# princeton-computational-imaging/Neural-Volume-Super-Resolution

Hardware: AMD Instinct MI355X
Metric: rendered rays/sec (64+128 samples) at 800x800 Lego-like view (higher is better)
Workload: dtype f32 as 2 f16 limbs (3 MFMA products, f32 acc); 1 GPU; Blender-'lego'-like 800x800 view, 64 coarse + 128 fine samples, tri-plane decoder (3x800^2x48 + 32^2x48 planes, 4+4x128 MLP), 1 view per GPU per step; partition=view

## Files before the change

neural-volume-super-resolution_amd/csrc/pair_core.h:

```cpp
#pragma once
#include <type_traits>
#include <utility>

#ifndef R3_DMA_AUX
#define R3_DMA_AUX 0
#endif
#ifndef R3_ABLATE
#define R3_ABLATE 0
#endif
#include "limb_core.h"
#include "side_work.h"

#ifndef R3_GATHER_NT
#define R3_GATHER_NT 0
#endif
#ifndef R3_STAMP
#define R3_STAMP 0
#endif
#if R3_STAMP == 4
#define R3_MARK(i)
#define R3_MARKB(i)
#define R3_RESET
#define R3_MARKH(i) { __builtin_amdgcn_sched_barrier(0); const unsigned long long t_ = __builtin_amdgcn_s_memtime(); stamp[i] += (float)(t_ - tprev); tprev = t_; __builtin_amdgcn_sched_barrier(0); }
#define R3_RESETH { tprev = __builtin_amdgcn_s_memtime(); }
#elif R3_STAMP == 3
#define R3_MARKH(i)
#define R3_RESETH
#define R3_MARK(i)
#define R3_MARKB(i) { __builtin_amdgcn_sched_barrier(0); const unsigned long long t_ = __builtin_amdgcn_s_memtime(); stamp[i] += (float)(t_ - tprev); tprev = t_; __builtin_amdgcn_sched_barrier(0); }
#define R3_RESET { tprev = __builtin_amdgcn_s_memtime(); }
#elif R3_STAMP
#define R3_MARKB(i)
#define R3_RESET
#define R3_MARKH(i)
#define R3_RESETH
#define R3_MARK(i) { __builtin_amdgcn_sched_barrier(0); const unsigned long long t_ = __builtin_amdgcn_s_memtime(); stamp[i] += (float)(t_ - tprev); tprev = t_; __builtin_amdgcn_sched_barrier(0); }
#else
#define R3_MARK(i)
#define R3_MARKB(i)
#define R3_RESET
#define R3_MARKH(i)
#define R3_RESETH
#endif
#ifndef R3_RELU_PK
#define R3_RELU_PK 0
#endif
#ifndef R3_BLEND_PK
#define R3_BLEND_PK 0
#endif
#ifndef R3_NO_VIEW_HOIST
#define R3_NO_VIEW_HOIST 1
#endif

namespace nvsr {

template <int LIMBS>
struct Lds3 {
    static constexpr bool F16 = limb_f16(LIMBS);
    static constexpr int SLOT = 4 * kb_words(LIMBS);
    static constexpr int SMALL = 2 * SLOT;
    static constexpr int RAYS = SMALL + SMALL_FLOATS;
    static constexpr int RAY_FLOATS = F16 ? 8 : 20;
    static constexpr int TAP_FLOATS = F16 ? 8 : 0;
    static constexpr int VTAPS = RAYS + RAYS2 * RAY_FLOATS;
    static constexpr int FAR = F16 ? VTAPS + RAYS2 * TAP_FLOATS : -1;
    static constexpr int RES = VTAPS + RAYS2 * TAP_FLOATS + (F16 ? RAYS2 : 0);
    static constexpr int RES_KB = F16 ? 9 : 0;
    static constexpr int PTS_WORDS = 8 * RAYS2;
    static constexpr int PTS = F16 ? VTAPS : RES + RES_KB * kb_words(LIMBS);
    static_assert(!F16 || RAYS2 * TAP_FLOATS >= PTS_WORDS, "the points' region fits the taps'");
    static constexpr int TOTAL = RES + RES_KB * kb_words(LIMBS) + (F16 ? 0 : PTS_WORDS);
};
static_assert(Lds3<3>::TOTAL * 4 <= 160 * 1024 && Lds3<2>::TOTAL * 4 <= 160 * 1024 && Lds3<1>::TOTAL * 4 <= 160 * 1024, "LDS budget");

struct Tile3 {
    f32x16 acc[4];
    f32x16 act[4];
    float D[HALF_C], F[HALF_C];
    float V[HALF_C];
    float T, cr, cg, cb, dep, ac, zc, zn;
    float raw[4];
};

struct RawTaps4 { f32x4 r[4][HALF_C / 4]; };
constexpr int GATHER_STEPS = 12 + HALF_C;
__device__ __forceinline__ void gather4_load(int k, const GatherJob& job, int h, RawTaps4& rt) {
    const int tap = k / 3, i0 = 2 * (k % 3);
#if R3_ABLATE & 1
    rt.r[tap][i0] = f32x4{job.t.nw, job.t.ne, job.t.sw, job.t.se};
    rt.r[tap][i0 + 1] = f32x4{job.t.se, job.t.ne, job.t.sw, job.t.nw};
    return;
#endif
    const int off = tap == 0 ? job.t.o00 : tap == 1 ? job.t.o01 : tap == 2 ? job.t.o10 : job.t.o11;
    const f32x4* p = reinterpret_cast<const f32x4*>(job.plane + off + HALF_C * h);
    rt.r[tap][i0] = p[i0];
    rt.r[tap][i0 + 1] = p[i0 + 1];
}
__device__ __forceinline__ void gather4_blend(int c, const GatherJob& job, const RawTaps4& rt, float (&F)[HALF_C]) {
    const int i = c >> 2, j = c & 3;
    F[c] = fmaf(rt.r[3][i][j], job.t.se, fmaf(rt.r[2][i][j], job.t.sw, fmaf(rt.r[1][i][j], job.t.ne, rt.r[0][i][j] * job.t.nw)));
}

template <int NS, bool LOADS, bool BLENDS, bool PK = false>
__device__ __forceinline__ void gather_roll(int slot, const GatherJob& jl, float (&Fl)[HALF_C], const GatherJob& jb, float (&Fb)[HALF_C], int h,
                                            RawTaps4& rt) {
    spread<72, 0, NS>(slot, [&](int v) {
        if (LOADS && v % 3 == 0) {
            const int tap = (v / 3) / 6, piece = (v / 3) % 6;
#if R3_ABLATE & 1
            rt.r[tap][piece] = f32x4{jl.t.nw, jl.t.ne, jl.t.sw, jl.t.se};
#else
            int off = tap == 0 ? jl.t.o00 : tap == 1 ? jl.t.o01 : tap == 2 ? jl.t.o10 : jl.t.o11;
#if R3_ABLATE & 2
            off = __builtin_amdgcn_readfirstlane(off);
#endif
#if R3_ABLATE & 4
            off = off & 0xffff;
            off -= off % 48;
#endif
#if R3_GATHER_NT
            rt.r[tap][piece] = __builtin_nontemporal_load(reinterpret_cast<const f32x4*>(jl.plane + off + HALF_C * h) + piece);
#else
            rt.r[tap][piece] = reinterpret_cast<const f32x4*>(jl.plane + off + HALF_C * h)[piece];
#endif
#endif
        }
        const int w = v / 18, u = v % 18;
        if constexpr (PK) {
            if (u % 3 != 2) {
                const int c = 2 * ((u / 3) * 2 + u % 3);
                if (LOADS && w == 3) {
                    f32x2_t m = f32x2_t{rt.r[0][c >> 2][c & 3], rt.r[0][c >> 2][(c & 3) + 1]} * f32x2_t{jl.t.nw, jl.t.nw};
                    Fl[c] = m[0]; Fl[c + 1] = m[1];
                }
                if (BLENDS && w < 3) {
                    const float wt = w == 0 ? jb.t.ne : w == 1 ? jb.t.sw : jb.t.se;
                    f32x2_t f = f32x2_t{Fb[c], Fb[c + 1]};
                    f32x2_t m = __builtin_elementwise_fma(f32x2_t{rt.r[w + 1][c >> 2][c & 3], rt.r[w + 1][c >> 2][(c & 3) + 1]}, f32x2_t{wt, wt}, f);
                    Fb[c] = m[0]; Fb[c + 1] = m[1];
                }
            }
        } else {
#pragma unroll
        for (int c = (u * 4) / 3; c < ((u + 1) * 4) / 3; ++c) {
            if (LOADS && w == 3) Fl[c] = rt.r[0][c >> 2][c & 3] * jl.t.nw;
            if (BLENDS && w < 3) Fb[c] = fmaf(rt.r[w + 1][c >> 2][c & 3], w == 0 ? jb.t.ne : w == 1 ? jb.t.sw : jb.t.se, Fb[c]);
        }
        }
    });
}

template <int NS, bool LOADS, int HL, bool BLENDS, int HB>
__device__ __forceinline__ void gather_half(int slot, const GatherJob& jl, const GatherJob& jb, float (&F)[HALF_C], int h, RawTaps2& rt) {
    if constexpr (BLENDS)
        spread<HALF_C, 0, NS / 2>(slot, [&](int c) {
            const float a = rt.r0[c >> 2][c & 3], b = rt.r1[c >> 2][c & 3];
            if (HB == 0) F[c] = fmaf(b, jb.t.ne, a * jb.t.nw);
            else F[c] = fmaf(b, jb.t.se, fmaf(a, jb.t.sw, F[c]));
        });
    if constexpr (LOADS)
        spread<12, NS / 2, NS>(slot, [&](int k) {
            const int off = HL == 0 ? ((k & 1) ? jl.t.o01 : jl.t.o00) : ((k & 1) ? jl.t.o11 : jl.t.o10);
            const f32x4 v = reinterpret_cast<const f32x4*>(jl.plane + off + HALF_C * h)[k >> 1];
            if (k & 1) rt.r1[k >> 1] = v; else rt.r0[k >> 1] = v;
        });
}

template <int N>
__device__ __forceinline__ void ring3_sync() {
#if R3_ABLATE & 256
#elif R3_ABLATE & 9
    asm volatile("s_waitcnt vmcnt(0)" ::: "memory");
#else
    asm volatile("s_waitcnt vmcnt(%0)" ::"n"(N) : "memory");
#endif
#if !(R3_ABLATE & 64)
    __syncthreads();
#endif
}

constexpr int RELU_STEPS = 68;
#ifndef R3_BOUNCE
#define R3_BOUNCE 0
#endif
typedef __attribute__((address_space(3))) f32x4* lds_f32x4_p;
struct BiasPend4 { f32x4 v[2]; f32x4 a[2]; lds_f32x4_p slot; };
__device__ __forceinline__ lds_f32x4_p bounce_slot(float* p) { return (lds_f32x4_p)p; }
template <int LIMBS>
__device__ __forceinline__ void relu_bias_step(int k, const float* bias, int h, const f32x16 (&acc)[4], f32x16 (&act)[4], BiasPend4& pend, f32x2_t nsc) {
    if ((k & 3) == 0 && k < 64) pend.v[(k >> 2) & 1] = *reinterpret_cast<const f32x4*>(bias + (k >> 2) * 8 + h * 4);
#if R3_BOUNCE
    if constexpr (LIMBS == 2) {
        if ((k & 3) == 0 && k < 64) {
            const int q = k >> 2;
            *pend.slot = f32x4{acc[q >> 2][4 * (q & 3)], acc[q >> 2][4 * (q & 3) + 1], acc[q >> 2][4 * (q & 3) + 2], acc[q >> 2][4 * (q & 3) + 3]};
        }
        if ((k & 3) == 2 && k < 66) {
            asm volatile("" : "+v"(pend.slot));
            pend.a[(k >> 2) & 1] = *pend.slot;
        }
        if (k >= 4) {
            const int r = k - 4;
            float v;
            asm("v_fma_f32 %0, -%1, %2, %3\n\tv_max_i32 %0, 0, %0" : "=v"(v) : "v"(pend.a[(r >> 2) & 1][r & 3]), "s"(nsc[0]), "v"(pend.v[(r >> 2) & 1][r & 3]));
            act[r >> 4][r & 15] = v;
        }
        return;
    }
#endif
#if R3_ABLATE & 2048
    if (k >= 4 && ((k - 4) & 15) != 0) return;
#endif
    if (k >= 4) {
        const int r = k - 4;
        if constexpr (LIMBS == 1) {
            float v, t;
            asm("v_mul_f32 %1, 0, %2\n\tv_fma_f32 %0, -%2, %3, %4\n\tv_add_f32 %0, %0, |%1|\n\tv_max_i32 %0, 0, %0"
                : "=v"(v), "=&v"(t) : "v"(acc[r >> 4][r & 15]), "s"(nsc[0]), "v"(pend.v[(r >> 2) & 1][r & 3]));
            act[r >> 4][r & 15] = v;
        } else if constexpr (LIMBS == 2) {
// ... 84 lines not shown
```

neural-volume-super-resolution_amd/csrc/render3.hip:

```cpp
#include "pair_core.h"

#include "colour_order.h"
#include "occupancy.h"
#include "nvsr_internal.h"

namespace nvsr {

template <int LZ>
__device__ __forceinline__ void render_pass3_body(const SceneDev& sc, const float* __restrict__ packed, long N, int S,
                                                  const float* __restrict__ rays, const float* __restrict__ z, int lindisp,
                                                  const float* __restrict__ noise, int white,
                                                  float* __restrict__ rgb, float* __restrict__ disp,
                                                  float* __restrict__ acc, float* __restrict__ weights,
                                                  float* __restrict__ depth, float* __restrict__ raw_out, unsigned* __restrict__ flag,
                                                  float* __restrict__ live_z = nullptr, float* __restrict__ live_w = nullptr,
                                                  int* __restrict__ live_n = nullptr, const int* __restrict__ group_slot = nullptr,
                                                  const int* __restrict__ pts = nullptr, const int* __restrict__ pt_steps = nullptr, float* views = nullptr,
                                                  const int* __restrict__ kept = nullptr, const int* __restrict__ kept_n = nullptr) {
    constexpr int LIMBS = LZ & 7;
    constexpr bool ZCOMP = (LZ & 8) != 0;
    constexpr int PHASE = (LZ >> 4) & 7;
    constexpr bool FUSED = PHASE == 0, KEPT = PHASE == 4, DENSITY = PHASE == 1 || KEPT, POINTS = PHASE == 3, COLOUR = PHASE == 2 || POINTS;
    constexpr bool F16 = limb_f16(LIMBS);
    using L = Lds3<LIMBS>;
// ... 76 lines not shown
        if constexpr (ZCOMP) return nullptr;
        asm volatile("" : "+v"(ray));
        return z + ray * S;
    };
    int idxX = 0, idxY = 0, idxXn = 0, idxYn = 0, cX = 0, cY = 0;
    bool actX = false, actY = false;
    auto kept_at = [&](const int* kp, int k, int prev) NVSR_INL -> int { const int e = kp[k < S ? k : S - 1]; return e < 0 ? prev : e; };
    auto live_depth = [&](const float* lzp, const float* rc, int n, int k) NVSR_INL -> float {
        if (n == 0) return rc[7];
        const float e = lzp[k < n ? k : n - 1];
        if constexpr (ZCOMP) return depth_of(nullptr, rc, __float_as_int(e));
        else return e;
    };
    auto live_weight = [](const float* lwp, int n, int k) NVSR_INL -> float { return n == 0 ? 0.0f : lwp[k < n ? k : n - 1]; };
    int slotX = ownX, slotY = ownY, slotXn = ownX, slotYn = ownY, eX1 = POINT_NONE, eY1 = POINT_NONE;
    bool liveX = false, liveY = false, liveXn = false, liveYn = false;
    float* const pt_sums = ldsf + L::PTS;
    float* const pt_exch = pt_sums + 3 * RAYS2;
    int* const pt_slot = reinterpret_cast<int*>(pt_exch + 3 * RAYS2);
    int* const pt_ray = pt_slot + RAYS2;
    const long pt_block = (long)(blk / (ORDER_RAYS / RAYS2)) * ORDER_RAYS;
    const int* const peX = POINTS ? pts + (long)blk * RAYS2 * S + ownX : nullptr;
    auto point_of = [&](int e, int own, int& slot, bool& live, float& zv, float& wv) NVSR_INL {
        live = e != POINT_NONE;
        slot = live ? (int)((unsigned)e >> 24) : own;
        const float* rc = ldsf + L::RAYS + slot * RAY3_FLOATS;
        zv = rc[7]; wv = 0.0f;
        if (live) {
            const long at = (pt_block + pt_ray[slot]) * S + (e & 0xffffff);
            const float ze = live_z[at];
            wv = live_w[at];
            if constexpr (ZCOMP) zv = coarse_depth(rc[7], L::FAR >= 0 ? ldsf[L::FAR + slot] : rc[16], __float_as_int(ze), S, lindisp);
            else zv = ze;
        }
    };
    auto load_view = [&](int slot, float (&V)[HALF_C]) NVSR_INL {
        const f32x4* vp = reinterpret_cast<const f32x4*>(views + ((long)blk * RAYS2 + slot) * POINT_VIEW_FLOATS + HALF_C * (lane0 >> 5));
#pragma unroll
        for (int i = 0; i < HALF_C / 4; ++i) { const f32x4 v = vp[i]; V[4 * i] = v[0]; V[4 * i + 1] = v[1]; V[4 * i + 2] = v[2]; V[4 * i + 3] = v[3]; }
    };
    if constexpr (POINTS) {
        static_assert(!R3_BOUNCE, "the points' LDS region is the f16 kernels' bounce slot");
        trip = __builtin_amdgcn_readfirstlane(pt_steps[blk]);
        __syncthreads();
    } else if constexpr (COLOUR || KEPT) {
        __shared__ int trip_s[NW2];
        int m = max(nX, nY);
#pragma unroll
        for (int o = 16; o >= 1; o >>= 1) m = max(m, __shfl_xor(m, o));
        if (lane0 == 0) trip_s[rs.wave] = m;
        __syncthreads();
        trip = __builtin_amdgcn_readfirstlane(max(max(trip_s[0], trip_s[1]), max(trip_s[2], trip_s[3])));
        if constexpr (KEPT) {
            const int* kX = kept_row(rayX);
            const int* kY = kept_row(rayY);
            actX = nX > 0; actY = nY > 0;
            idxX = kept_at(kX, 0, 0); idxY = kept_at(kY, 0, 0);
            idxXn = kept_at(kX, 1, idxX); idxYn = kept_at(kY, 1, idxY);
            X.zc = depth_of(z_row(rayX), rcX, idxX); Y.zc = depth_of(z_row(rayY), rcY, idxY);
        } else {
            X.zc = live_depth(lzX, rcX, nX, 0); Y.zc = live_depth(lzY, rcY, nY, 0);
            wX = live_weight(lwX, nX, 0); wY = live_weight(lwY, nY, 0);
        }
    } else {
        if constexpr (ZCOMP) __syncthreads();
        X.zc = depth_of(zX, rcX, 0); Y.zc = depth_of(zY, rcY, 0);
    }
    RawTaps4 rt;
    RawTaps2 r2;

    auto point_norm = [&](const float* rc, float zc, float& n0, float& n1, float& n2) NVSR_INL {
        const f32x4 c0 = reinterpret_cast<const f32x4*>(rc)[0], c1 = reinterpret_cast<const f32x4*>(rc)[1];
        n0 = norm_coord(__fadd_rn(c0[0], __fmul_rn(c0[3], zc)), sc.lo[0], sc.range[0]);
        n1 = norm_coord(__fadd_rn(c0[1], __fmul_rn(c1[0], zc)), sc.lo[1], sc.range[1]);
        n2 = norm_coord(__fadd_rn(c0[2], __fmul_rn(c1[1], zc)), sc.lo[2], sc.range[2]);
    };
    auto scale_taps = [](Taps& t) NVSR_INL {
        if constexpr (F16) { t.nw *= F16_X_SCALE; t.ne *= F16_X_SCALE; t.sw *= F16_X_SCALE; t.se *= F16_X_SCALE; }
    };
    auto view_job = [&](const float* rtp) NVSR_INL {
        const f32x4 c2 = reinterpret_cast<const f32x4*>(rtp)[0], c3 = reinterpret_cast<const f32x4*>(rtp)[1];
        GatherJob j;
        j.plane = sc.plane[3];
        j.t.o00 = __float_as_int(c2[0]); j.t.o01 = __float_as_int(c2[1]); j.t.o10 = __float_as_int(c2[2]); j.t.o11 = __float_as_int(c2[3]);
        j.t.nw = c3[0]; j.t.ne = c3[1]; j.t.sw = c3[2]; j.t.se = c3[3];
        scale_taps(j.t);
        return j;
    };

    __syncthreads();
    if constexpr (!DENSITY) {
#pragma unroll
        for (int k2 = 0; k2 < 2; ++k2) {
            Tile3& t = k2 ? Y : X;
            const GatherJob vj = view_job(k2 ? rtY : rtX);
#pragma unroll
            for (int k = 0; k < 12; ++k) gather4_load(k, vj, lane0 >> 5, rt);
#pragma unroll
            for (int c = 0; c < HALF_C; ++c) gather4_blend(c, vj, rt, t.V);
        }
        if constexpr (POINTS) {
#pragma unroll
            for (int k2 = 0; k2 < 2; ++k2) {
                const Tile3& t = k2 ? Y : X;
                f32x4* vp = reinterpret_cast<f32x4*>(views + ((long)blk * RAYS2 + (k2 ? ownY : ownX)) * POINT_VIEW_FLOATS + HALF_C * (lane0 >> 5));
#pragma unroll
                for (int i = 0; i < HALF_C / 4; ++i) vp[i] = f32x4{t.V[4 * i], t.V[4 * i + 1], t.V[4 * i + 2], t.V[4 * i + 3]};
            }
            __syncthreads();
            if (lane0 < 32) {
#pragma unroll
                for (int c = 0; c < 3; ++c) pt_sums[ownX * 3 + c] = pt_sums[ownY * 3 + c] = 0.0f;
                pt_ray[ownX] = (int)(rayX - pt_block); pt_ray[ownY] = (int)(rayY - pt_block);
            }
            __syncthreads();
            const int eX0 = trip > 0 ? peX[0] : POINT_NONE, eY0 = trip > 0 ? peX[32] : POINT_NONE;
            eX1 = trip > 1 ? peX[RAYS2] : POINT_NONE; eY1 = trip > 1 ? peX[RAYS2 + 32] : POINT_NONE;
            point_of(eX0, ownX, slotX, liveX, X.zc, wX);
            point_of(eY0, ownY, slotY, liveY, Y.zc, wY);
            load_view(slotX, X.V); load_view(slotY, Y.V);
        }
    } else {
#pragma unroll
        for (int k2 = 0; k2 < 2; ++k2) {
            Tile3& t = k2 ? Y : X;
            float n0, n1, n2;
            point_norm(k2 ? rcY : rcX, t.zc, n0, n1, n2);
#pragma unroll
            for (int p = 0; p < 3; ++p) {
                GatherJob pj;
                pj.plane = sc.plane[p]; pj.t = pos_taps2(sc, p, n0, n1, n2); scale_taps(pj.t);
#pragma unroll
                for (int k = 0; k < 12; ++k) gather4_load(k, pj, lane0 >> 5, rt);
#pragma unroll
                for (int c = 0; c < HALF_C; ++c) gather4_blend(c, pj, rt, t.F);
#pragma unroll
                for (int c = 0; c < HALF_C; ++c) {
                    t.D[c] = p == 0 ? t.F[c] : p == 1 ? __fadd_rn(t.D[c], t.F[c]) : div3(__fadd_rn(t.D[c], t.F[c]));
                    asm volatile("" : "+v"(t.D[c]));
                }
                __builtin_amdgcn_sched_barrier(0);
            }
        }
    }
    auto head_out = [](float v) NVSR_INL { if constexpr (LIMBS == 1) return fabsf(v) == __builtin_inff() ? __builtin_nanf("") : v; else return v; };
    Limbs<LIMBS> cur, fa;
    f32x2_t nsc = {-F16_ACC_UNSCALE, -F16_ACC_UNSCALE};
    asm volatile("" : "+s"(nsc));
#if R3_STAMP
    float stamp[8] = {0, 0, 0, 0, 0, 0, 0, 0};
    unsigned long long tprev = __builtin_amdgcn_s_memtime();
#endif
    constexpr bool RESIDENT = L::RES_KB > 0 && !DENSITY;
    constexpr int KB_FIRST = DENSITY ? KB_DEN0 : RESIDENT ? KB_RGB0 + 9 : KB_RGB0;
    unsigned* const res = lds + L::RES;
    if constexpr (RESIDENT) ring3_load_resident<LIMBS, L::RES_KB>(rs, res, KB_RGB0);
    unsigned* cw = const_cast<unsigned*>(ring3_issue<LIMBS, 3>(rs, KB_FIRST));
    const int steps = COLOUR || KEPT ? trip : S;
    for (int s = 0; s < steps; ++s) {
        asm volatile("" : "+v"(rs.voff), "+v"(rs.lane));
#if R3_NO_VIEW_HOIST
        if constexpr (!POINTS) {
#pragma unroll
        for (int c = 0; c < HALF_C; ++c) asm volatile("" : "+v"(X.V[c]), "+v"(Y.V[c]));
        }
#endif
        if constexpr (POINTS) { rcX = ldsf + L::RAYS + slotX * RAY3_FLOATS; rcY = ldsf + L::RAYS + slotY * RAY3_FLOATS; }
        const int lane = rs.lane, h = lane >> 5;
        const bool last = (s + 1 == S);
        if constexpr (!COLOUR && !KEPT) {
            X.zn = depth_of(zX, rcX, last ? s : s + 1);
            Y.zn = depth_of(zY, rcY, last ? s : s + 1);
        }
        const float nzX = !COLOUR && noise ? noise[rayX * S + s] : 0.0f;
        const float nzY = !COLOUR && noise ? noise[rayY * S + s] : 0.0f;
        float xn0, xn1, xn2, yn0, yn1, yn2;
        if constexpr (!KEPT) {
            point_norm(rcX, DENSITY ? X.zn : X.zc, xn0, xn1, xn2);
            point_norm(rcY, DENSITY ? Y.zn : Y.zc, yn0, yn1, yn2);
        }
        BiasPend4 bp;
        bp.slot = bounce_slot(ldsf + L::VTAPS + rs.wave * 64 * L::TAP_FLOATS + lane * 4);
        HeadPend<3> hp3;
        HeadPend<1> hp1;
        SplitPend tp;

        auto feat = [](const float (&f)[HALF_C]) NVSR_INL { return [&f](int kb, int i) NVSR_INL { return f[8 * kb + i]; }; };
        auto hid = [](const f32x16 (&a)[4], int kb0) NVSR_INL { return [&a, kb0](int kb, int i) NVSR_INL { const int k = kb0 + kb; return a[k >> 1][8 * (k & 1) + i]; }; };
        auto split_feat = [&](const float (&f)[HALF_C]) NVSR_INL { split_all<LIMBS>([&f](int i) NVSR_INL { return f[i]; }, cur); };
        auto tail_of = [&](const f32x16 (&a)[4], int kb) NVSR_INL {
            return [&a, kb, &tp](int slice, Limbs<LIMBS>& nxt) NVSR_INL { split_slice<LIMBS>(slice, [&a, kb](int i) NVSR_INL { return a[kb >> 1][8 * (kb & 1) + i]; }, nxt, tp); };
        };
        auto none = [](int) NVSR_INL {};

        GatherJob ja, jb;
        R3_MARK(0)
        ring3_sync<(ZCOMP || COLOUR || KEPT) ? 0 : 2>();
        int eX2 = POINT_NONE, eY2 = POINT_NONE;
        if constexpr (POINTS) {
            if (s + 2 < steps) { eX2 = peX[(s + 2) * RAYS2]; eY2 = peX[(s + 2) * RAYS2 + 32]; }
            point_of(eX1, ownX, slotXn, liveXn, X.zn, wXn);
            point_of(eY1, ownY, slotYn, liveYn, Y.zn, wYn);
        } else if constexpr (COLOUR) {
            X.zn = live_depth(lzX, rcX, nX, s + 1); Y.zn = live_depth(lzY, rcY, nY, s + 1);
            wXn = live_weight(lwX, nX, s + 1); wYn = live_weight(lwY, nY, s + 1);
        } else if constexpr (KEPT) {
            X.zn = depth_of(z_row(rayX), rcX, idxXn); Y.zn = depth_of(z_row(rayY), rcY, idxYn);
            point_norm(rcX, X.zn, xn0, xn1, xn2);
            point_norm(rcY, Y.zn, yn0, yn1, yn2);
        }
        unsigned* nw = (RESIDENT || DENSITY) ? nullptr : ring3_take(rs);
        float hx[3] = {0.0f, 0.0f, 0.0f};
        if constexpr (!DENSITY) {
        const unsigned* const w_view = RESIDENT ? res : cw;
        R3_MARK(1)
        R3_RESET
#define NVSR_ROLL(TL, JL, TB, JB, LOADS, BLENDS) [&](int slot) NVSR_INL { gather_roll<NSF, LOADS, BLENDS, F16 && R3_BLEND_PK>(slot, JL, TL.F, JB, TB.F, h, rt); }
#define NVSR_ROLL_DMA(TL, JL, TB, JB, LOADS, BLENDS, NKB, KB0) \
        [&](int slot) NVSR_INL { gather_roll<NSF, LOADS, BLENDS, F16 && R3_BLEND_PK>(slot, JL, TL.F, JB, TB.F, h, rt); dma_side<LIMBS, NKB>(slot, rs, nw, KB0); }
        ja.plane = sc.plane[0]; ja.t = pos_taps2(sc, 0, xn0, xn1, xn2); scale_taps(ja.t);
        split_feat(X.V);
        if constexpr (RESIDENT) limb_block<LIMBS, 3, true, true>(w_view, lane, X.acc, cur, fa, feat(X.V), NVSR_ROLL(X, ja, Y, jb, true, false), NoTail{});
        else limb_block<LIMBS, 3, true, true>(cw, lane, X.acc, cur, fa, feat(X.V), NVSR_ROLL_DMA(X, ja, Y, jb, true, false, 3, KB_RGB0 + 3), NoTail{});
        R3_MARKB(0)
        if constexpr (POINTS) load_view(slotXn, X.V);
        jb.plane = sc.plane[0]; jb.t = pos_taps2(sc, 0, yn0, yn1, yn2); scale_taps(jb.t);
        split_feat(Y.V);
        limb_block<LIMBS, 3, true, false>(w_view, lane, Y.acc, cur, fa, feat(Y.V), NVSR_ROLL(Y, jb, X, ja, true, true), NoTail{});
        R3_MARKB(1)
        if constexpr (POINTS) load_view(slotYn, Y.V);
        const unsigned* w_p0 = res + 3 * kb_words(LIMBS);
        if constexpr (!RESIDENT) {
            cw = nw;
            ring3_sync<YOUNGER_THAN_CHUNK>();
            nw = ring3_take(rs);
            w_p0 = cw;
        }
#pragma unroll
        for (int c = 0; c < HALF_C; ++c) X.D[c] = X.F[c];
        ja.plane = sc.plane[1]; ja.t = pos_taps2(sc, 1, xn0, xn1, xn2); scale_taps(ja.t);
        split_feat(X.F);
        if constexpr (RESIDENT) limb_block<LIMBS, 3, false, true>(w_p0, lane, X.acc, cur, fa, feat(X.F), NVSR_ROLL(X, ja, Y, jb, true, true), NoTail{});
        else limb_block<LIMBS, 3, false, true>(cw, lane, X.acc, cur, fa, feat(X.F), NVSR_ROLL_DMA(X, ja, Y, jb, true, true, 3, KB_RGB0 + 6), NoTail{});
        R3_MARKB(2)
#pragma unroll
        for (int c = 0; c < HALF_C; ++c) Y.D[c] = Y.F[c];
        jb.plane = sc.plane[1]; jb.t = pos_taps2(sc, 1, yn0, yn1, yn2); scale_taps(jb.t);
        split_feat(Y.F);
        limb_block<LIMBS, 3, false, false>(w_p0, lane, Y.acc, cur, fa, feat(Y.F), NVSR_ROLL(Y, jb, X, ja, true, true), NoTail{});
        R3_MARKB(3)
        const unsigned* w_p1 = res + 6 * kb_words(LIMBS);
        if constexpr (!RESIDENT) {
            cw = nw;
            ring3_sync<YOUNGER_THAN_CHUNK>();
            nw = ring3_take(rs);
            w_p1 = cw;
        }
#pragma unroll
        for (int c = 0; c < HALF_C; ++c) X.D[c] = __fadd_rn(X.D[c], X.F[c]);
        ja.plane = sc.plane[2]; ja.t = pos_taps2(sc, 2, xn0, xn1, xn2); scale_taps(ja.t);
        split_feat(X.F);
        if constexpr (RESIDENT) limb_block<LIMBS, 3, false, true>(w_p1, lane, X.acc, cur, fa, feat(X.F), NVSR_ROLL(X, ja, Y, jb, true, true), NoTail{});
        else limb_block<LIMBS, 3, false, true>(cw, lane, X.acc, cur, fa, feat(X.F), NVSR_ROLL_DMA(X, ja, Y, jb, true, true, 3, KB_RGB0 + 9), NoTail{});
        R3_MARKB(4)
#pragma unroll
        for (int c = 0; c < HALF_C; ++c) Y.D[c] = __fadd_rn(Y.D[c], Y.F[c]);
        jb.plane = sc.plane[2]; jb.t = pos_taps2(sc, 2, yn0, yn1, yn2); scale_taps(jb.t);
        split_feat(Y.F);
        limb_block<LIMBS, 3, false, false>(w_p1, lane, Y.acc, cur, fa, feat(Y.F), NVSR_ROLL(Y, jb, X, ja, true, true), NoTail{});
        R3_MARKB(5)
        if constexpr (!RESIDENT) {
            cw = nw;
            ring3_sync<YOUNGER_THAN_CHUNK>();
        }
        nw = ring3_take(rs);
#pragma unroll
        for (int c = 0; c < HALF_C; ++c) X.D[c] = div3(__fadd_rn(X.D[c], X.F[c]));
        split_feat(X.F);
        limb_block<LIMBS, 3, false, true>(cw, lane, X.acc, cur, fa, feat(X.F), NVSR_ROLL_DMA(X, ja, Y, jb, false, true, 4, KB_RGB1), NoTail{});
        R3_MARKB(6)
#pragma unroll
        for (int c = 0; c < HALF_C; ++c) Y.D[c] = div3(__fadd_rn(Y.D[c], Y.F[c]));
        split_feat(Y.F);
        limb_block<LIMBS, 3, false, false>(cw, lane, Y.acc, cur, fa, feat(Y.F),
                                           [&](int slot) NVSR_INL { spread<RELU_STEPS, 0, NSF>(slot, [&](int k) NVSR_INL { relu_bias_step<LIMBS>(k, small + S_BIAS + 4 * HID, h, X.acc, X.act, bp, nsc); }); },
                                           tail_of(X.act, 0));
        R3_MARKB(7)
        cw = nw;
        R3_MARK(2)
        }

        auto relu_side = [&](Tile3& t, int bias_vec) NVSR_INL {
            return [&, bias_vec](int slot) NVSR_INL { spread<RELU_STEPS, 0, NSH>(slot, [&](int k) NVSR_INL { relu_bias_step<LIMBS>(k, small + S_BIAS + bias_vec * HID, h, t.acc, t.act, bp, nsc); }); };
        };
#define NVSR_HIDDEN_LAYER_(SYNC, XA_SIDE, VPREV, VTHIS, KB_NEXT_A, NKB_A, KB_NEXT_B, NKB_B, X_B_SIDE)                                \
        R3_RESETH                                                                                                                   \
        SYNC;                                                                                                                       \
        R3_MARKH(0)                                                                                                                 \
        nw = ring3_take(rs);                                                                                                        \
        R3_MARKH(1)                                                                                                                 \
        limb_block<LIMBS, 4, true, true>(cw, lane, X.acc, cur, fa, hid(X.act, 0),                                                   \
                                         [&](int slot) NVSR_INL { (XA_SIDE)(slot); dma_side<LIMBS, NKB_A>(slot, rs, nw, KB_NEXT_A); }, tail_of(Y.act, 0)); \
        R3_MARKH(2)                                                                                                                 \
        limb_block<LIMBS, 4, true, false>(cw, lane, Y.acc, cur, fa, hid(Y.act, 0), none, tail_of(X.act, 4));                        \
        R3_MARKH(3)                                                                                                                 \
        cw = nw;                                                                                                                    \
        ring3_sync<0>();                                                                                                               \
        nw = ring3_take(rs);                                                                                                        \
        R3_MARKH(4)                                                                                                                 \
        limb_block<LIMBS, 4, false, true>(cw, lane, X.acc, cur, fa, hid(X.act, 4),                                                  \
                                          [&](int slot) NVSR_INL { dma_side<LIMBS, NKB_B>(slot, rs, nw, KB_NEXT_B); }, tail_of(Y.act, 4));   \
        R3_MARKH(5)                                                                                                                 \
        X_B_SIDE;                                                                                                                   \
        R3_MARKH(6)                                                                                                                 \
        cw = nw;

#define NVSR_HIDDEN_LAYER(VPREV, ...) NVSR_HIDDEN_LAYER_(ring3_sync<0>(), relu_side(Y, VPREV), VPREV, __VA_ARGS__)
#define NVSR_YB_PLAIN(VTHIS) (limb_block<LIMBS, 4, false, false>(cw, lane, Y.acc, cur, fa, hid(Y.act, 4), relu_side(X, VTHIS), tail_of(X.act, 0)))
        if constexpr (!DENSITY) {
        NVSR_HIDDEN_LAYER(4, 5, KB_RGB1 + 4, 4, KB_RGB1 + 8, 4, NVSR_YB_PLAIN(5))
        NVSR_HIDDEN_LAYER(5, 6, KB_RGB1 + 12, 4, KB_RGB1 + 16, 4, NVSR_YB_PLAIN(6))
        NVSR_HIDDEN_LAYER(6, 7, KB_RGB1 + 20, 4, (COLOUR ? KB_FIRST : KB_DEN0), 3,
                          (limb_block<LIMBS, 4, false, false>(cw, lane, Y.acc, cur, fa, hid(Y.act, 4),
                                                              [&](int slot) NVSR_INL {
                                                                  if constexpr (COLOUR) {
                                                                      spread<RELU_STEPS, 0, NSH / 2>(slot, [&](int k) NVSR_INL { relu_bias_step<LIMBS>(k, small + S_BIAS + 7 * HID, h, X.acc, X.act, bp, nsc); });
                                                                      spread<64, NSH / 2, NSH>(slot, [&](int k) NVSR_INL { heads_side<3>(k >> 2, k & 3, small + S_RGB_W, h, X.act, hx, hp3); });
                                                                  } else relu_side(X, 7)(slot);
                                                              },
                                                              NoTail{})))
        }

        R3_MARK(3)
        if constexpr (FUSED) {
        ring3_sync<0>();
        nw = ring3_take(rs);
        split_feat(X.D);
        limb_block<LIMBS, 3, true, true>(cw, lane, X.acc, cur, fa, feat(X.D),
                                         [&](int slot) NVSR_INL {
                                             spread<RELU_STEPS, 0, NSF>(slot, [&](int k) NVSR_INL { relu_bias_step<LIMBS>(k, small + S_BIAS + 7 * HID, h, Y.acc, Y.act, bp, nsc); });
                                             spread<64, 0, NSF>(slot, [&](int k) NVSR_INL { heads_side<3>(k >> 2, k & 3, small + S_RGB_W, h, X.act, hx, hp3); });
                                             dma_side<LIMBS, 4>(slot, rs, nw, KB_DEN1);
                                         },
                                         NoTail{});
#pragma unroll
        for (int c = 0; c < 3; ++c) X.raw[c] = head_out((hx[c] + __shfl_xor(hx[c], 32)) + small[S_HEAD_B + 1 + c]);
        float hy[3] = {0.0f, 0.0f, 0.0f};
        split_feat(Y.D);
        limb_block<LIMBS, 3, true, false>(cw, lane, Y.acc, cur, fa, feat(Y.D),
                                          [&](int slot) NVSR_INL {
                                              spread<64, 0, NSF>(slot, [&](int k) NVSR_INL { heads_side<3>(k >> 2, k & 3, small + S_RGB_W, h, Y.act, hy, hp3); });
                                              spread<RELU_STEPS, 0, NSF>(slot, [&](int k) NVSR_INL { relu_bias_step<LIMBS>(k, small + S_BIAS + 0 * HID, h, X.acc, X.act, bp, nsc); });
                                          },
                                          tail_of(X.act, 0));
#pragma unroll
        for (int c = 0; c < 3; ++c) Y.raw[c] = head_out((hy[c] + __shfl_xor(hy[c], 32)) + small[S_HEAD_B + 1 + c]);
        cw = nw;

        R3_MARK(4)
        NVSR_HIDDEN_LAYER(0, 1, KB_DEN1 + 4, 4, KB_DEN1 + 8, 4, NVSR_YB_PLAIN(1))
        NVSR_HIDDEN_LAYER(1, 2, KB_DEN1 + 12, 4, KB_DEN1 + 16, 4, NVSR_YB_PLAIN(2))
        } else if constexpr (DENSITY) {
        float (&Fg)[HALF_C] = X.F;
#define NVSR_HALF(JL, HL, JB, HB, LOADS, BLENDS, NS_) gather_half<NS_, LOADS, HL, BLENDS, HB>(slot, JL, JB, Fg, h, r2)
#define NVSR_JOB(J, P, N0, N1, N2) J.plane = sc.plane[P]; J.t = pos_taps2(sc, P, N0, N1, N2); scale_taps(J.t);
        nw = ring3_take(rs);
        NVSR_JOB(ja, 0, xn0, xn1, xn2)
        split_feat(X.D);
        limb_block<LIMBS, 3, true, true>(cw, lane, X.acc, cur, fa, feat(X.D),
                                         [&](int slot) NVSR_INL { NVSR_HALF(ja, 0, ja, 0, true, false, NSF); dma_side<LIMBS, 4>(slot, rs, nw, KB_DEN1); }, NoTail{});
        split_feat(Y.D);
        limb_block<LIMBS, 3, true, false>(cw, lane, Y.acc, cur, fa, feat(Y.D),
                                          [&](int slot) NVSR_INL {
                                              spread<RELU_STEPS, 0, NSF>(slot, [&](int k) NVSR_INL { relu_bias_step<LIMBS>(k, small + S_BIAS + 0 * HID, h, X.acc, X.act, bp, nsc); });
                                              NVSR_HALF(ja, 1, ja, 0, true, true, NSF);
                                          },
                                          tail_of(X.act, 0));
        cw = nw;
#define NVSR_DEN_LAYER(VPREV, KB_NEXT_A, KB_NEXT_B, NKB_B, PRE_XA, G_XA, PRE_YA, G_YA, PRE_XB, G_XB, PRE_YB, YB_SIDE, YB_TAIL)                      \
        ring3_sync<12>();                                                                                                           \
        nw = ring3_take(rs);                                                                                                        \
        PRE_XA                                                                                                                      \
        limb_block<LIMBS, 4, true, true>(cw, lane, X.acc, cur, fa, hid(X.act, 0),                                                   \
                                         [&](int slot) NVSR_INL { relu_side(Y, VPREV)(slot); G_XA; dma_side<LIMBS, 4>(slot, rs, nw, KB_NEXT_A); }, tail_of(Y.act, 0)); \
        PRE_YA                                                                                                                      \
        limb_block<LIMBS, 4, true, false>(cw, lane, Y.acc, cur, fa, hid(Y.act, 0), [&](int slot) NVSR_INL { G_YA; }, tail_of(X.act, 4)); \
        cw = nw;                                                                                                                    \
        ring3_sync<12>();                                                                                                           \
        nw = ring3_take(rs);                                                                                                        \
        PRE_XB                                                                                                                      \
        limb_block<LIMBS, 4, false, true>(cw, lane, X.acc, cur, fa, hid(X.act, 4),                                                  \
                                          [&](int slot) NVSR_INL { G_XB; dma_side<LIMBS, NKB_B>(slot, rs, nw, KB_NEXT_B); }, tail_of(Y.act, 4)); \
        PRE_YB                                                                                                                      \
        limb_block<LIMBS, 4, false, false>(cw, lane, Y.acc, cur, fa, hid(Y.act, 4), [&](int slot) NVSR_INL { YB_SIDE; }, YB_TAIL);     \
        cw = nw;
#define NVSR_D_SET(T) _Pragma("unroll") for (int c = 0; c < HALF_C; ++c) { T.D[c] = Fg[c]; asm volatile("" : "+v"(T.D[c])); }
#define NVSR_D_ADD(T) _Pragma("unroll") for (int c = 0; c < HALF_C; ++c) { T.D[c] = __fadd_rn(T.D[c], Fg[c]); asm volatile("" : "+v"(T.D[c])); }
#define NVSR_D_AVG(T) _Pragma("unroll") for (int c = 0; c < HALF_C; ++c) { T.D[c] = div3(__fadd_rn(T.D[c], Fg[c])); asm volatile("" : "+v"(T.D[c])); }
        NVSR_DEN_LAYER(0, KB_DEN1 + 4, KB_DEN1 + 8, 4,
                       NVSR_JOB(jb, 1, xn0, xn1, xn2), NVSR_HALF(jb, 0, ja, 1, true, true, NSH),
                       NVSR_D_SET(X), NVSR_HALF(jb, 1, jb, 0, true, true, NSH),
                       NVSR_JOB(ja, 2, xn0, xn1, xn2), NVSR_HALF(ja, 0, jb, 1, true, true, NSH),
                       NVSR_D_ADD(X), relu_side(X, 1)(slot); NVSR_HALF(ja, 1, ja, 0, true, true, NSH), tail_of(X.act, 0))
        NVSR_DEN_LAYER(1, KB_DEN1 + 12, KB_DEN1 + 16, 4,
                       NVSR_JOB(jb, 0, yn0, yn1, yn2), NVSR_HALF(jb, 0, ja, 1, true, true, NSH),
                       NVSR_D_AVG(X), NVSR_HALF(jb, 1, jb, 0, true, true, NSH),
                       NVSR_JOB(ja, 1, yn0, yn1, yn2), NVSR_HALF(ja, 0, jb, 1, true, true, NSH),
                       NVSR_D_SET(Y), relu_side(X, 2)(slot); NVSR_HALF(ja, 1, ja, 0, true, true, NSH), tail_of(X.act, 0))
        float sx[1] = {0.0f};
        auto sigma_side = [&](int slot) NVSR_INL {
            spread<RELU_STEPS, 0, NSH / 2>(slot, [&](int k) NVSR_INL { relu_bias_step<LIMBS>(k, small + S_BIAS + 3 * HID, h, X.acc, X.act, bp, nsc); });
            spread<64, NSH / 2, NSH>(slot, [&](int k) NVSR_INL { heads_side<1>(k >> 2, k & 3, small + S_ALPHA_W, h, X.act, sx, hp1); });
        };
        NVSR_DEN_LAYER(2, KB_DEN1 + 20, KB_FIRST, 3,
                       NVSR_JOB(jb, 2, yn0, yn1, yn2), NVSR_HALF(jb, 0, ja, 1, true, true, NSH),
                       NVSR_D_ADD(Y), NVSR_HALF(jb, 1, jb, 0, true, true, NSH),
                       , NVSR_HALF(jb, 1, jb, 1, false, true, NSH),
                       NVSR_D_AVG(Y), sigma_side(slot), NoTail{})
#undef NVSR_DEN_LAYER
#undef NVSR_D_SET
#undef NVSR_D_ADD
#undef NVSR_D_AVG
#undef NVSR_HALF
#undef NVSR_JOB
        X.raw[3] = head_out((sx[0] + __shfl_xor(sx[0], 32)) + small[S_HEAD_B]);
        }
        if constexpr (FUSED) {
        float sx[1] = {0.0f};
        NVSR_HIDDEN_LAYER(2, 3, KB_DEN1 + 20, 4, KB_FIRST, 3,
                          (limb_block<LIMBS, 4, false, false>(cw, lane, Y.acc, cur, fa, hid(Y.act, 4),
                                                              [&](int slot) NVSR_INL {
                                                                  spread<RELU_STEPS, 0, NSH / 2>(slot, [&](int k) NVSR_INL { relu_bias_step<LIMBS>(k, small + S_BIAS + 3 * HID, h, X.acc, X.act, bp, nsc); });
                                                                  spread<64, NSH / 2, NSH>(slot, [&](int k) NVSR_INL { heads_side<1>(k >> 2, k & 3, small + S_ALPHA_W, h, X.act, sx, hp1); });
                                                              },
                                                              NoTail{})))
        X.raw[3] = head_out((sx[0] + __shfl_xor(sx[0], 32)) + small[S_HEAD_B]);
        }
        R3_MARK(5)
        if constexpr (!COLOUR) {

        float zsX = 0.0f, zsY = 0.0f;
        int e1X = 0, e1Y = 0, e2X = 0, e2Y = 0;
        const bool lastX = KEPT ? idxX + 1 == S : last, lastY = KEPT ? idxY + 1 == S : last;
        if constexpr (KEPT) {
            zsX = depth_of(z_row(rayX), rcX, lastX ? idxX : idxX + 1); zsY = depth_of(z_row(rayY), rcY, lastY ? idxY : idxY + 1);
            { const int* kX = kept_row(rayX); e1X = kX[s + 1 < S ? s + 1 : S - 1]; e2X = kX[s + 2 < S ? s + 2 : S - 1]; }
            { const int* kY = kept_row(rayY); e1Y = kY[s + 1 < S ? s + 1 : S - 1]; e2Y = kY[s + 2 < S ? s + 2 : S - 1]; }
        }
#pragma unroll
        for (int k = 0; k < RELU_STEPS; ++k) relu_bias_step<LIMBS>(k, small + S_BIAS + 3 * HID, h, Y.acc, Y.act, bp, nsc);
        {
            float hd[1];
            head_dots<1>(small + S_ALPHA_W, h, Y.act, hd);
            Y.raw[3] = head_out(hd[0] + small[S_HEAD_B]);
        }
        if (raw_out && lane < 32) {
            if (validX) *reinterpret_cast<f32x4*>(raw_out + (rayX * S + s) * 4) = f32x4{X.raw[0], X.raw[1], X.raw[2], X.raw[3]};
            if (validY) *reinterpret_cast<f32x4*>(raw_out + (rayY * S + s) * 4) = f32x4{Y.raw[0], Y.raw[1], Y.raw[2], Y.raw[3]};
        }
        if constexpr (!KEPT) actX = actY = true;
        if constexpr (KEPT) {
            {
                const float t0 = X.T, d0 = X.dep, a0 = X.ac, g0 = X.zn;
                X.zn = zsX;
                composite_weight(X, reinterpret_cast<const f32x4*>(rcX)[1][2], 0.0f, lastX);
                X.zn = g0; X.T = actX ? X.T : t0; X.dep = actX ? X.dep : d0; X.ac = actX ? X.ac : a0;
            }
            {
                const float t0 = Y.T, d0 = Y.dep, a0 = Y.ac, g0 = Y.zn;
                Y.zn = zsY;
                composite_weight(Y, reinterpret_cast<const f32x4*>(rcY)[1][2], 0.0f, lastY);
                Y.zn = g0; Y.T = actY ? Y.T : t0; Y.dep = actY ? Y.dep : d0; Y.ac = actY ? Y.ac : a0;
            }
        } else if constexpr (DENSITY) {
            composite_weight(X, reinterpret_cast<const f32x4*>(rcX)[1][2], nzX, last);
            composite_weight(Y, reinterpret_cast<const f32x4*>(rcY)[1][2], nzY, last);
        } else {
            composite_sample(X, reinterpret_cast<const f32x4*>(rcX)[1][2], nzX, last);
            composite_sample(Y, reinterpret_cast<const f32x4*>(rcY)[1][2], nzY, last);
        }
        if (weights && lane < 32) {
            if (validX && actX) weights[rayX * S + (KEPT ? idxX : s)] = X.raw[3];
            if (validY && actY) weights[rayY * S + (KEPT ? idxY : s)] = Y.raw[3];
        }
        if constexpr (DENSITY) {
            const bool liveX = actX && !(X.raw[3] == 0.0f), liveY = actY && !(Y.raw[3] == 0.0f);
            if (lane < 32) {
                if (validX && liveX) { live_z[rayX * S + cX] = ZCOMP ? __int_as_float(KEPT ? idxX : s) : X.zc; live_w[rayX * S + cX] = X.raw[3]; }
                if (validY && liveY) { live_z[rayY * S + cY] = ZCOMP ? __int_as_float(KEPT ? idxY : s) : Y.zc; live_w[rayY * S + cY] = Y.raw[3]; }
            }
            cX += liveX; cY += liveY;
            if constexpr (KEPT) {
                actX = validX && s + 1 < S && e1X >= 0; actY = validY && s + 1 < S && e1Y >= 0;
                idxX = e1X < 0 ? idxX : e1X; idxY = e1Y < 0 ? idxY : e1Y;
                idxXn = e2X < 0 ? idxX : e2X; idxYn = e2Y < 0 ? idxY : e2Y;
            }
        }
        } else {
#pragma unroll
        for (int c = 0; c < 3; ++c) X.raw[c] = head_out((hx[c] + __shfl_xor(hx[c], 32)) + small[S_HEAD_B + 1 + c]);
#pragma unroll
        for (int k = 0; k < RELU_STEPS; ++k) relu_bias_step<LIMBS>(k, small + S_BIAS + 7 * HID, h, Y.acc, Y.act, bp, nsc);
        {
            float hd[3];
            head_dots<3>(small + S_RGB_W, h, Y.act, hd);
#pragma unroll
            for (int c = 0; c < 3; ++c) Y.raw[c] = head_out(hd[c] + small[S_HEAD_B + 1 + c]);
        }
        if constexpr (POINTS) {
            if (lane < 32) {
#pragma unroll
                for (int c = 0; c < 3; ++c) { pt_exch[ownX * 3 + c] = colour_term(wX, X.raw[c]); pt_exch[ownY * 3 + c] = colour_term(wY, Y.raw[c]); }
                pt_slot[ownX] = liveX ? slotX : -1; pt_slot[ownY] = liveY ? slotY : -1;
            }
            __syncthreads();
            const int p = rs.wave * 64 + lane, sl = pt_slot[p];
            if (sl >= 0 && (p == 0 || pt_slot[p - 1] != sl)) {
                float a0 = pt_sums[sl * 3], a1 = pt_sums[sl * 3 + 1], a2 = pt_sums[sl * 3 + 2];
                int q = p;
                do {
                    a0 = __fadd_rn(a0, pt_exch[q * 3]); a1 = __fadd_rn(a1, pt_exch[q * 3 + 1]); a2 = __fadd_rn(a2, pt_exch[q * 3 + 2]);
                    ++q;
                } while (q < RAYS2 && pt_slot[q] == sl);
                pt_sums[sl * 3] = a0; pt_sums[sl * 3 + 1] = a1; pt_sums[sl * 3 + 2] = a2;
            }
            __syncthreads();
            slotX = slotXn; slotY = slotYn; liveX = liveXn; liveY = liveYn; eX1 = eX2; eY1 = eY2;
        } else {
            composite_colour(X, wX, s < nX);
            composite_colour(Y, wY, s < nY);
        }
        wX = wXn; wY = wYn;
        }
#undef NVSR_HIDDEN_LAYER
#undef NVSR_HIDDEN_LAYER_
#undef NVSR_ROLL
#undef NVSR_ROLL_DMA
#undef NVSR_YB_PLAIN
        X.zc = X.zn; Y.zc = Y.zn;
        R3_MARK(6)
    }
#if R3_STAMP
    if (raw_out && rs.lane < 32 && validX) {
        for (int i = 0; i < 8; ++i) raw_out[(rayX * S + (i >> 2)) * 4 + (i & 3)] = stamp[i] / (float)S;
    }
#endif
    asm volatile("s_waitcnt vmcnt(0)" ::: "memory");

    if constexpr (POINTS) {
        if (rs.lane < 32) {
            X.cr = pt_sums[ownX * 3]; X.cg = pt_sums[ownX * 3 + 1]; X.cb = pt_sums[ownX * 3 + 2];
            Y.cr = pt_sums[ownY * 3]; Y.cg = pt_sums[ownY * 3 + 1]; Y.cb = pt_sums[ownY * 3 + 2];
        }
    }
    if (rs.lane < 32) {
#pragma unroll
        for (int k = 0; k < 2; ++k) {
            const Tile3& t = k ? Y : X;
            const long ray = k ? rayY : rayX;
            if (!(k ? validY : validX)) continue;
            float cr = t.cr, cg = t.cg, cb = t.cb;
            const float ac = COLOUR ? acc[ray] : t.ac;
            if constexpr (!COLOUR) {
                const float q = t.dep / t.ac;
                disp[ray] = 1.0f / ((q != q) ? q : fmaxf(1e-10f, q));
                acc[ray] = t.ac;
                if (depth) depth[ray] = t.dep;
// ... 303 lines not shown
```

Baseline: 8.126 million rays/s.

## Keep first nine density-MLP K-blocks resident in LDS for two-limb path

For the two-limb density pass, the first nine weight K-blocks (layer 0 plus most of layer 1's first chunk) are loaded once into the resident LDS region instead of being streamed through the ring every step. Layer 0 and part of layer 1 then read from resident LDS, the per-step ring sync at the top of the loop is dropped, and the ring's first fetch and the wrap-around issue at layer 2 start later at the remaining blocks. This aims to cut per-step weight DMA and ring waits, at the cost of a hand-split layer-1 schedule with reshuffled gather/relu side work and different sync counts.

```diff
diff --git a/neural-volume-super-resolution_amd/csrc/pair_core.h b/neural-volume-super-resolution_amd/csrc/pair_core.h
--- a/neural-volume-super-resolution_amd/csrc/pair_core.h
+++ b/neural-volume-super-resolution_amd/csrc/pair_core.h
@@ -66,6 +66,9 @@
     static constexpr int FAR = F16 ? VTAPS + RAYS2 * TAP_FLOATS : -1;
     static constexpr int RES = VTAPS + RAYS2 * TAP_FLOATS + (F16 ? RAYS2 : 0);
     static constexpr int RES_KB = F16 ? 9 : 0;
+    static constexpr int DEN_RES_KB = LIMBS == 2 ? RES_KB : 0;
+    static constexpr int DEN_CHUNK_KB = 4;
+    static_assert(DEN_CHUNK_KB * kb_words(LIMBS) == SLOT, "the density ring is the ring");
     static constexpr int PTS_WORDS = 8 * RAYS2;
     static constexpr int PTS = F16 ? VTAPS : RES + RES_KB * kb_words(LIMBS);
     static_assert(!F16 || RAYS2 * TAP_FLOATS >= PTS_WORDS, "the points' region fits the taps'");
diff --git a/neural-volume-super-resolution_amd/csrc/render3.hip b/neural-volume-super-resolution_amd/csrc/render3.hip
--- a/neural-volume-super-resolution_amd/csrc/render3.hip
+++ b/neural-volume-super-resolution_amd/csrc/render3.hip
@@ -252,10 +252,15 @@
     unsigned long long tprev = __builtin_amdgcn_s_memtime();
 #endif
     constexpr bool RESIDENT = L::RES_KB > 0 && !DENSITY;
-    constexpr int KB_FIRST = DENSITY ? KB_DEN0 : RESIDENT ? KB_RGB0 + 9 : KB_RGB0;
+    constexpr bool DRES = DENSITY && L::DEN_RES_KB > 0;
+    static_assert(!DRES || L::DEN_RES_KB == 9, "the split of layer 1 chunk b below is written for 3 + 4 + 2 resident K-blocks");
+    constexpr int KB_FIRST = DRES ? KB_DEN0 + L::DEN_RES_KB : DENSITY ? KB_DEN0 : RESIDENT ? KB_RGB0 + 9 : KB_RGB0;
+    constexpr int NKB_FIRST = DRES ? KB_DEN1 + 8 - KB_FIRST : 3;
     unsigned* const res = lds + L::RES;
     if constexpr (RESIDENT) ring3_load_resident<LIMBS, L::RES_KB>(rs, res, KB_RGB0);
-    unsigned* cw = const_cast<unsigned*>(ring3_issue<LIMBS, 3>(rs, KB_FIRST));
+    if constexpr (DRES) ring3_load_resident<LIMBS, L::DEN_RES_KB>(rs, res, KB_DEN0);
+    unsigned* cw = const_cast<unsigned*>(ring3_issue<LIMBS, NKB_FIRST>(rs, KB_FIRST));
+    if constexpr (DRES) ring3_sync<NKB_FIRST * LIMBS>();
     const int steps = COLOUR || KEPT ? trip : S;
     for (int s = 0; s < steps; ++s) {
         asm volatile("" : "+v"(rs.voff), "+v"(rs.lane));
@@ -295,7 +300,7 @@
 
         GatherJob ja, jb;
         R3_MARK(0)
-        ring3_sync<(ZCOMP || COLOUR || KEPT) ? 0 : 2>();
+        if constexpr (!DRES) ring3_sync<(ZCOMP || COLOUR || KEPT) ? 0 : 2>();
         int eX2 = POINT_NONE, eY2 = POINT_NONE;
         if constexpr (POINTS) {
             if (s + 2 < steps) { eX2 = peX[(s + 2) * RAYS2]; eY2 = peX[(s + 2) * RAYS2 + 32]; }
@@ -464,19 +469,24 @@
         float (&Fg)[HALF_C] = X.F;
 #define NVSR_HALF(JL, HL, JB, HB, LOADS, BLENDS, NS_) gather_half<NS_, LOADS, HL, BLENDS, HB>(slot, JL, JB, Fg, h, r2)
 #define NVSR_JOB(J, P, N0, N1, N2) J.plane = sc.plane[P]; J.t = pos_taps2(sc, P, N0, N1, N2); scale_taps(J.t);
-        nw = ring3_take(rs);
+        const unsigned* const w_d0 = DRES ? res : cw;
+        if constexpr (!DRES) nw = ring3_take(rs);
         NVSR_JOB(ja, 0, xn0, xn1, xn2)
         split_feat(X.D);
-        limb_block<LIMBS, 3, true, true>(cw, lane, X.acc, cur, fa, feat(X.D),
-                                         [&](int slot) NVSR_INL { NVSR_HALF(ja, 0, ja, 0, true, false, NSF); dma_side<LIMBS, 4>(slot, rs, nw, KB_DEN1); }, NoTail{});
+        limb_block<LIMBS, 3, true, true>(w_d0, lane, X.acc, cur, fa, feat(X.D),
+                                         [&](int slot) NVSR_INL {
+                                             NVSR_HALF(ja, 0, ja, 0, true, false, NSF);
+                                             if constexpr (!DRES) dma_side<LIMBS, 4>(slot, rs, nw, KB_DEN1);
+                                         },
+                                         NoTail{});
         split_feat(Y.D);
-        limb_block<LIMBS, 3, true, false>(cw, lane, Y.acc, cur, fa, feat(Y.D),
+        limb_block<LIMBS, 3, true, false>(w_d0, lane, Y.acc, cur, fa, feat(Y.D),
                                           [&](int slot) NVSR_INL {
                                               spread<RELU_STEPS, 0, NSF>(slot, [&](int k) NVSR_INL { relu_bias_step<LIMBS>(k, small + S_BIAS + 0 * HID, h, X.acc, X.act, bp, nsc); });
                                               NVSR_HALF(ja, 1, ja, 0, true, true, NSF);
                                           },
                                           tail_of(X.act, 0));
-        cw = nw;
+        if constexpr (!DRES) cw = nw;
 #define NVSR_DEN_LAYER(VPREV, KB_NEXT_A, KB_NEXT_B, NKB_B, PRE_XA, G_XA, PRE_YA, G_YA, PRE_XB, G_XB, PRE_YB, YB_SIDE, YB_TAIL)                      \
         ring3_sync<12>();                                                                                                           \
         nw = ring3_take(rs);                                                                                                        \
@@ -497,11 +507,44 @@
 #define NVSR_D_SET(T) _Pragma("unroll") for (int c = 0; c < HALF_C; ++c) { T.D[c] = Fg[c]; asm volatile("" : "+v"(T.D[c])); }
 #define NVSR_D_ADD(T) _Pragma("unroll") for (int c = 0; c < HALF_C; ++c) { T.D[c] = __fadd_rn(T.D[c], Fg[c]); asm volatile("" : "+v"(T.D[c])); }
 #define NVSR_D_AVG(T) _Pragma("unroll") for (int c = 0; c < HALF_C; ++c) { T.D[c] = div3(__fadd_rn(T.D[c], Fg[c])); asm volatile("" : "+v"(T.D[c])); }
+        if constexpr (DRES) {
+            const unsigned* const w_1a = res + 3 * kb_words(LIMBS);
+            const unsigned* const w_1b = res + 7 * kb_words(LIMBS);
+            NVSR_JOB(jb, 1, xn0, xn1, xn2)
+            limb_block<LIMBS, 4, true, true>(w_1a, lane, X.acc, cur, fa, hid(X.act, 0),
+                                             [&](int slot) NVSR_INL { relu_side(Y, 0)(slot); NVSR_HALF(jb, 0, ja, 1, true, true, NSH); }, tail_of(Y.act, 0));
+            NVSR_D_SET(X)
+            limb_block<LIMBS, 4, true, false>(w_1a, lane, Y.acc, cur, fa, hid(Y.act, 0), [&](int slot) NVSR_INL { NVSR_HALF(jb, 1, jb, 0, true, true, NSH); },
+                                              tail_of(X.act, 4));
+            NVSR_JOB(ja, 2, xn0, xn1, xn2)
+            limb_block<LIMBS, 2, false, true>(w_1b, lane, X.acc, cur, fa, hid(X.act, 4), [&](int slot) NVSR_INL { NVSR_HALF(ja, 0, jb, 1, true, true, NSH); },
+                                              tail_of(X.act, 6));
+            ring3_sync<48>();
+            nw = ring3_take(rs);
+            limb_block<LIMBS, 2, false, true>(cw, lane, X.acc, cur, fa, hid(X.act, 6),
+                                              [&](int sl) NVSR_INL {
+                                                  const int slot = sl + NSH / 2;
+                                                  NVSR_HALF(ja, 0, jb, 1, true, true, NSH);
+                                                  dma_side<LIMBS, 4>(sl, rs, nw, KB_DEN1 + 8);
+                                              },
+                                              tail_of(Y.act, 4));
+            NVSR_D_ADD(X)
+            limb_block<LIMBS, 2, false, true>(w_1b, lane, Y.acc, cur, fa, hid(Y.act, 4),
+                                              [&](int slot) NVSR_INL { relu_side(X, 1)(slot); NVSR_HALF(ja, 1, ja, 0, true, true, NSH); }, tail_of(Y.act, 6));
+            limb_block<LIMBS, 2, false, true>(cw, lane, Y.acc, cur, fa, hid(Y.act, 6),
+                                              [&](int sl) NVSR_INL {
+                                                  const int slot = sl + NSH / 2;
+                                                  relu_side(X, 1)(slot); NVSR_HALF(ja, 1, ja, 0, true, true, NSH);
+                                              },
+                                              tail_of(X.act, 0));
+            cw = nw;
+        } else {
         NVSR_DEN_LAYER(0, KB_DEN1 + 4, KB_DEN1 + 8, 4,
                        NVSR_JOB(jb, 1, xn0, xn1, xn2), NVSR_HALF(jb, 0, ja, 1, true, true, NSH),
                        NVSR_D_SET(X), NVSR_HALF(jb, 1, jb, 0, true, true, NSH),
                        NVSR_JOB(ja, 2, xn0, xn1, xn2), NVSR_HALF(ja, 0, jb, 1, true, true, NSH),
                        NVSR_D_ADD(X), relu_side(X, 1)(slot); NVSR_HALF(ja, 1, ja, 0, true, true, NSH), tail_of(X.act, 0))
+        }
         NVSR_DEN_LAYER(1, KB_DEN1 + 12, KB_DEN1 + 16, 4,
                        NVSR_JOB(jb, 0, yn0, yn1, yn2), NVSR_HALF(jb, 0, ja, 1, true, true, NSH),
                        NVSR_D_AVG(X), NVSR_HALF(jb, 1, jb, 0, true, true, NSH),
@@ -512,7 +555,7 @@
             spread<RELU_STEPS, 0, NSH / 2>(slot, [&](int k) NVSR_INL { relu_bias_step<LIMBS>(k, small + S_BIAS + 3 * HID, h, X.acc, X.act, bp, nsc); });
             spread<64, NSH / 2, NSH>(slot, [&](int k) NVSR_INL { heads_side<1>(k >> 2, k & 3, small + S_ALPHA_W, h, X.act, sx, hp1); });
         };
-        NVSR_DEN_LAYER(2, KB_DEN1 + 20, KB_FIRST, 3,
+        NVSR_DEN_LAYER(2, KB_DEN1 + 20, KB_FIRST, NKB_FIRST,
                        NVSR_JOB(jb, 2, yn0, yn1, yn2), NVSR_HALF(jb, 0, ja, 1, true, true, NSH),
                        NVSR_D_ADD(Y), NVSR_HALF(jb, 1, jb, 0, true, true, NSH),
                        , NVSR_HALF(jb, 1, jb, 1, false, true, NSH),
```

New measurement: 8.249 million rays/s (median of 6 runs). 1.02x the previous value.
